# ocrickard/piper-swift

Hardware: AMD Instinct MI355X
Metric: audio-sec/wall-sec (RTF^-1) with ms/utterance, Piper VITS en_GB-medium geometry, scale-bench factor (higher is better)
Workload: dtype f32; 1 GPU; medium factor=8: 112 ids, 336 frames, 86016 samples (3.901 s audio) per utterance, 1 utterance per step per GPU; factor=8, phoneme_count=112, frames=336, samples=86016, parallelism=utterance-replicas x1 (one-shot RCCL weight broadcast)

## Files before the change

piper-swift_amd/csrc/rb_pair.hip:

```cpp
#include <algorithm>
#include <type_traits>

#include "conv_win.h"

namespace ph {
namespace {

typedef float f32x16 __attribute__((ext_vector_type(16)));

constexpr int kRA = 8;
constexpr int kStepPad = 16;
constexpr int kWN = 4, kNTW = 2, kT1 = kWN * kNTW;
constexpr int kColsA = 32 * kT1;
__host__ __device__ constexpr int halo_of(int pb) { return pb <= 16 ? 16 : 48; }
constexpr int kMaxReachB = 48;
constexpr int kStageU = 10;

struct RbPairMulti {
  RbPairArgs c[kWinMulti];
};

#ifdef PH_PAIR_TRACE
__device__ unsigned long long* ph_pair_trace_buf;
#define PH_STAMP(k) do { if (lane == 0 && round < 4 && ph_pair_trace_buf && blockIdx.x < 512) ph_pair_trace_buf[(((size_t)blockIdx.x * (MT * kWN) + wave) * 4 + round) * 8 + (k)] = __builtin_amdgcn_s_memtime(); } while (0)
#else
#define PH_STAMP(k) do { } while (0)
#endif

__device__ __forceinline__ float lrelu_max(float v, float alpha) { return fmaxf(v, v * alpha); }

__device__ __forceinline__ float bload(__amdgpu_buffer_rsrc_t r, int voff, int soff) {
  return __builtin_bit_cast(float, __builtin_amdgcn_raw_buffer_load_b32(r, voff, soff, 0));
}
__device__ __forceinline__ void bstore(__amdgpu_buffer_rsrc_t r, float v, int voff, int soff) {
  __builtin_amdgcn_raw_buffer_store_b32(__builtin_bit_cast(int, v), r, voff, soff, 0);
}

struct PairSched {
  int ntx[kWinMulti];
  int cnt[kWinMulti];
  int total, batch, order;
};

template <int MT>
__global__ __launch_bounds__(MT * kWN * 64, 2) void rb_pair_kernel(const RbPairMulti multi, const PairSched sch, const int Wx, const int W1,
                                                               const unsigned inv_w4) {
  extern __shared__ __attribute__((aligned(16))) float lds[];
  constexpr int BT = MT * kWN * 64;
  const int lane = threadIdx.x & 63;
  const int wave = __builtin_amdgcn_readfirstlane((int)(threadIdx.x >> 6));
  const int wm = wave % MT, wn = wave / MT;
  const int r = lane & 31, h = lane >> 5;
  constexpr int C = 32 * MT, C2 = C >> 1;
  float* xs = lds;
  float* x1s = lds + C * Wx + 4;
  float* biasS = x1s + C * W1;
  for (int i = threadIdx.x; i < kWinMulti * 2 * C; i += BT) {
    const int z = i / (2 * C), rem = i - z * 2 * C;
    const RbPairArgs& p = multi.c[(sch.order >> (4 * z)) & 15];
    biasS[i] = rem < C ? p.ba[rem] : p.bb[rem - C];
  }
  const int rowlane = wm * 32 + 4 * h;
  const unsigned lane16 = (unsigned)lane * 16u;
  const int G = (int)gridDim.x, bid = (int)blockIdx.x;

  struct Tile {
    const float *x, *wa4, *wb4;
    float* y;
    int bias_off;
    int Ka, dila, Kb, dilb, res_a, res_b_x, L, Lv, pa, pb, halo, c0, ga, shift, Sa, Spa, Sb, Spb, ntb;
    float alpha;
  };
  auto tile_index = [&](int round) {
    const int idx = round * G + ((round & 1) ? G - 1 - bid : bid);
    return idx < sch.total ? idx : -1;
  };
  auto setup = [&](int idx) {
    int z = 0, rem = idx;
    if (rem >= sch.cnt[0]) { rem -= sch.cnt[0]; z = 1; }
    if (z == 1 && rem >= sch.cnt[1]) { rem -= sch.cnt[1]; z = 2; }
    const RbPairArgs& p = multi.c[(sch.order >> (4 * z)) & 15];
    const int ntx = sch.ntx[z];
    const int n = __builtin_amdgcn_readfirstlane(rem / ntx);
    const int bx = rem - n * ntx;
    Tile t;
    t.x = p.x + (int64_t)n * C * p.L;
    t.y = p.y + (int64_t)n * C * p.L;
    t.wa4 = p.wa4; t.wb4 = p.wb4; t.bias_off = z * 2 * C;
    t.Ka = p.Ka; t.dila = p.dila; t.Kb = p.Kb; t.dilb = p.dilb; t.res_a = p.res_a; t.res_b_x = p.res_b_x; t.L = p.L; t.alpha = p.alpha;
    t.Lv = p.len_ptr ? min(p.len_ptr[n] * p.len_mul, p.L) : p.L;
    t.pa = (p.Ka - 1) * p.dila / 2; t.pb = (p.Kb - 1) * p.dilb / 2;
    t.halo = halo_of(t.pb);
    const int ncb = kColsA - 2 * t.halo;
    t.c0 = bx * ncb;
    const int g0 = t.c0 - t.halo - t.pa;
    t.ga = g0 & ~3;
    t.shift = g0 - t.ga;
    t.Sa = p.Ka * C2; t.Spa = (t.Sa + kStepPad - 1) / kStepPad * kStepPad;
    t.Sb = p.Kb * C2; t.Spb = (t.Sb + kStepPad - 1) / kStepPad * kStepPad;
    t.ntb = min(max((ncb >> 5) - wn * kNTW, 0), kNTW);
    return t;
  };

  float4 a[kRA];
  const char* wa = nullptr;
  auto load_a = [&](int slot, int ahead) { a[slot] = *(const float4*)(wa + ahead * 1024 + lane16); };
  auto ring_start = [&](const float* w4, int Sp) {
    wa = (const char*)w4 + (int64_t)wm * Sp * 256;
#pragma unroll
    for (int d = 0; d < kRA - 1; d++) load_a(d, d);
  };

  float4 pre[kStageU];
  const int W4 = Wx >> 2, total4 = C * W4;
  auto stage_issue = [&](const Tile& t, const int tx) {
#pragma unroll
    for (int u = 0; u < kStageU; u++) {
      const int ic = min(tx + u * BT, total4 - 1);
      const int row = (int)__umulhi((unsigned)ic, inv_w4);
      const int pos = t.ga + 4 * (ic - row * W4);
      pre[u] = *(const float4*)(t.x + (int64_t)row * t.L + ((pos >= 0 && pos < t.L) ? pos : 0));
    }
  };
  auto stage_commit = [&](const Tile& t, const int tx) {
#pragma unroll
    for (int u = 0; u < kStageU; u++) {
      const int i = tx + u * BT;
      const int ic = min(i, total4 - 1);
      const int row = (int)__umulhi((unsigned)ic, inv_w4);
      const int i4 = ic - row * W4;
      const int pos = t.ga + 4 * i4;
      const int nv = (pos >= 0 && pos < t.L) ? t.Lv - pos : 0;
      float4 v = pre[u];
      v.x = nv > 0 ? lrelu_max(v.x, t.alpha) : 0.0f; v.y = nv > 1 ? lrelu_max(v.y, t.alpha) : 0.0f;
      v.z = nv > 2 ? lrelu_max(v.z, t.alpha) : 0.0f; v.w = nv > 3 ? lrelu_max(v.w, t.alpha) : 0.0f;
      *(float4*)(xs + (i < total4 ? row * Wx + 4 * i4 : C * Wx)) = v;
    }
  };

  f32x16 acc[kNTW];
  auto run_conv = [&](auto nt_tag, const float* img, const int Wrow, const int S, const int Sp, const int dil, const int col0, const int bias_off) {
    constexpr int NT = decltype(nt_tag)::value;
#pragma unroll
    for (int g4 = 0; g4 < 4; g4++) {
      const float4 bv = *(const float4*)(biasS + bias_off + rowlane + 8 * g4);
#pragma unroll
      for (int j = 0; j < kNTW; j++) { acc[j][4 * g4] = bv.x; acc[j][4 * g4 + 1] = bv.y; acc[j][4 * g4 + 2] = bv.z; acc[j][4 * g4 + 3] = bv.w; }
    }
    const int lbase = h * Wrow + col0 + r;
    int sidx = 0, c_n = 0, left = S - 1;
    const int wrap_delta = dil - 2 * Wrow * (C2 - 1);
    float b[2][NT][4];
    auto read_b4 = [&](int slot) {
#pragma unroll
      for (int e = 0; e < 4; e++) {
#pragma unroll
        for (int j = 0; j < NT; j++) b[slot][j][e] = img[lbase + sidx + 32 * j];
        c_n++;
        const bool wrap = c_n == C2;
        c_n = wrap ? 0 : c_n;
        const int delta = wrap ? wrap_delta : 2 * Wrow;
        sidx += left > 0 ? delta : 0;
        left--;
      }
    };
    auto group = [&](int u) {
      load_a((u + kRA - 1) % kRA, kRA - 1 + u);
      read_b4((u + 1) & 1);
      __builtin_amdgcn_sched_barrier(0);
      const float av[4] = {a[u].x, a[u].y, a[u].z, a[u].w};
#pragma unroll
      for (int e = 0; e < 4; e++)
#pragma unroll
        for (int j = 0; j < NT; j++) acc[j] = __builtin_amdgcn_mfma_f32_32x32x2f32(av[e], b[u & 1][j][e], acc[j], 0, 0, 0);
    };
    read_b4(0);
    const int Gr = Sp >> 2, full = Gr / kRA;
    if (full > 0) {
#pragma unroll
      for (int u = 0; u < kRA; u++) group(u);
      wa += kRA * 1024;
    }
    for (int g = 1; g < full; g++) {
#pragma unroll
      for (int u = 0; u < kRA; u++) group(u);
      wa += kRA * 1024;
    }
    const int rem = Gr - full * kRA;
#pragma unroll
    for (int u = 0; u < kRA - 1; u++)
      if (u < rem) group(u);
  };

  Tile cur = setup(tile_index(0));
  ring_start(cur.wa4, cur.Spa);
  stage_issue(cur, (int)threadIdx.x);
  stage_commit(cur, (int)threadIdx.x);
  __syncthreads();

  for (int round = 0;; round++) {
    const int nidx = tile_index(round + 1);
    const bool has_next = nidx >= 0;
    const Tile nxt = has_next ? setup(nidx) : cur;
    int tx = (int)threadIdx.x, rl = rowlane, rr = r;
    asm volatile("" : "+v"(tx), "+v"(rl), "+v"(rr));
    float resx[kNTW][16];
    auto load_res = [&](int gres0) {
      const __amdgpu_buffer_rsrc_t rx = __builtin_amdgcn_make_buffer_rsrc((void*)cur.x, 0, C * cur.L * 4, 0x00020000);
#pragma unroll
      for (int j = 0; j < kNTW; j++) {
        const int g = gres0 + (wn * kNTW + j) * 32 + rr;
        const int voff = (g >= 0 && g < cur.L) ? (rl * cur.L + g) * 4 : -4;
#pragma unroll
        for (int q = 0; q < 16; q++) resx[j][q] = bload(rx, voff, ((q & 3) + 8 * (q >> 2)) * cur.L * 4);
      }
    };

    PH_STAMP(0);
    __builtin_amdgcn_s_waitcnt(0x0F70);
    PH_STAMP(1);
    if (has_next) stage_issue(nxt, tx);

    const bool live = cur.c0 < cur.Lv;
    if (live) run_conv(std::integral_constant<int, kNTW>{}, xs, Wx, cur.Sa, cur.Spa, cur.dila, cur.shift + wn * kNTW * 32, cur.bias_off);
    PH_STAMP(2);
    if (live) ring_start(cur.wb4, cur.Spb);
    if (live && cur.res_a) load_res(cur.c0 - cur.halo);
    __syncthreads();
    PH_STAMP(3);

    if (live) {
#pragma unroll
      for (int j = 0; j < kNTW; j++) {
        const int colw = (wn * kNTW + j) * 32 + rr;
        const int g = cur.c0 - cur.halo + colw;
        const bool in = g >= 0 && g < cur.Lv;
#pragma unroll
        for (int q = 0; q < 16; q++) {
          const int rq = (q & 3) + 8 * (q >> 2);
          const int o = (rl + rq) * W1 + colw;
          float v = acc[j][q];
          if (cur.res_a) v += resx[j][q];
          v = in ? v : 0.0f;
          x1s[o] = lrelu_max(v, cur.alpha);
          if (!cur.res_b_x) xs[o] = v;
        }
      }
    }
    __syncthreads();

    PH_STAMP(4);
    if (live && cur.ntb > 0) {
      const int col0b = cur.halo - cur.pb + wn * kNTW * 32;
      __builtin_amdgcn_s_waitcnt(0x0F70);
      if (cur.ntb == 2) run_conv(std::integral_constant<int, 2>{}, x1s, W1, cur.Sb, cur.Spb, cur.dilb, col0b, cur.bias_off + C);
      else run_conv(std::integral_constant<int, 1>{}, x1s, W1, cur.Sb, cur.Spb, cur.dilb, col0b, cur.bias_off + C);
    }
    PH_STAMP(5);
    if (has_next) ring_start(nxt.wa4, nxt.Spa);
    if (live && cur.res_b_x && cur.ntb > 0) load_res(cur.c0);
    if (live && cur.ntb > 0) {
      const __amdgpu_buffer_rsrc_t ry = __builtin_amdgcn_make_buffer_rsrc((void*)cur.y, 0, C * cur.L * 4, 0x00020000);
#pragma unroll
      for (int j = 0; j < kNTW; j++) {
        if (j >= cur.ntb) break;
        const int colo = (wn * kNTW + j) * 32 + rr;
        const int g = cur.c0 + colo;
        const int voff = g < cur.L ? (rl * cur.L + g) * 4 : -4;
#pragma unroll
        for (int q = 0; q < 16; q++) {
          const int rq = (q & 3) + 8 * (q >> 2);
          float v = acc[j][q];
          v += cur.res_b_x ? resx[j][q] : xs[(rl + rq) * W1 + cur.halo + colo];
          bstore(ry, v, voff, rq * cur.L * 4);
        }
      }
    }
    PH_STAMP(6);
    if (!has_next) break;
    __syncthreads();
    stage_commit(nxt, tx);
    __syncthreads();
    PH_STAMP(7);
    cur = nxt;
  }
}

struct PairGeom {
  int Wx, W1;
  size_t lds;
};

PairGeom pair_geom(int C, int pa_max, int pb_max) {
  auto pad = [](int w, bool odd32) {
    w = (w + 3) & ~3;
    if (odd32) while ((w & 63) != 32) w += 4;
    return w;
  };
  PairGeom g;
  for (int pass = 0; pass < 2; pass++) {
    g.Wx = pad(kColsA + 2 * pa_max + 3, pass == 0);
    g.W1 = pad(kColsA, pass == 0);
    (void)pb_max;
    g.lds = ((size_t)C * g.Wx + 4 + (size_t)C * g.W1 + (size_t)kWinMulti * 2 * C) * sizeof(float);
    if (g.lds <= 160 * 1024 && (C * g.Wx) / 4 <= kStageU * (C / 32) * kWN * 64) break;
  }
  return g;
}

template <int MT>
void launch_pair_inst(piper_hip_ctx* ctx, hipStream_t s, const RbPairMulti& m, const PairSched& sch, const PairGeom& g) {
  static bool raised[kMaxDevices] = {};
  if (g.lds > 64 * 1024 && lds_optin_needed(raised))
    (void)hipFuncSetAttribute((const void*)rb_pair_kernel<MT>, hipFuncAttributeMaxDynamicSharedMemorySize, 160 * 1024);
  const unsigned inv = (unsigned)(0x100000000ull / (unsigned)(g.Wx >> 2)) + 1u;
  const int per_cu = std::max(1, std::min(2, (int)((size_t)160 * 1024 / g.lds)));
  const int grid = std::min(sch.total, per_cu * ctx->num_cus);
  hipLaunchKernelGGL((rb_pair_kernel<MT>), dim3(grid), dim3(MT * kWN * 64), g.lds, s, m, sch, g.Wx, g.W1, inv);
}

}

#ifdef PH_PAIR_TRACE
void rb_pair_set_trace(unsigned long long* buf) { (void)hipMemcpyToSymbol(HIP_SYMBOL(ph_pair_trace_buf), &buf, sizeof buf); }
#endif

bool rb_pair_eligible(int C, int Ka, int dila, int Kb, int dilb, int L) {
  if (C != 32 && C != 64) return false;
  if (Ka < 1 || Kb < 1 || !(Ka & 1) || !(Kb & 1) || dila < 1 || dilb < 1) return false;
  if (L < 4 || (L & 3)) return false;
  const int pa = (Ka - 1) * dila / 2, pb = (Kb - 1) * dilb / 2;
  if (pb > kMaxReachB) return false;
  if ((int64_t)C * (kColsA + 2 * pa + 70) >= (1 << 20)) return false;
  const PairGeom g = pair_geom(C, pa, pb);
  return g.lds <= 160 * 1024 && (C * g.Wx) / 4 <= kStageU * (C / 32) * kWN * 64;
}

int launch_rb_pair_multi(piper_hip_ctx* ctx, hipStream_t s, const RbPairArgs* pairs, int count) {
  if (count < 1 || count > kWinMulti) PH_FAIL(PIPER_HIP_ERR_ARG, "rb_pair: %d pairs in one launch (1..%d)", count, kWinMulti);
  const RbPairArgs& a = pairs[0];
  if (a.N <= 0 || a.L <= 0) return PIPER_HIP_OK;
  int pa_max = 0, pb_max = 0;
  int idx[kWinMulti] = {0, 1, 2};
  for (int i = 0; i < count; i++) {
    const RbPairArgs& b = pairs[i];
    if (b.N != a.N || b.C != a.C || b.L != a.L) PH_FAIL(PIPER_HIP_ERR_SHAPE, "rb_pair: pairs of one launch must share N, C and L");
    if (!rb_pair_eligible(b.C, b.Ka, b.dila, b.Kb, b.dilb, b.L)) PH_FAIL(PIPER_HIP_ERR_UNSUPPORTED, "rb_pair: geometry not covered (C=%d K=%d,%d d=%d,%d L=%d)", b.C, b.Ka, b.Kb, b.dila, b.dilb, b.L);
    if (!(b.alpha > 0.0f && b.alpha < 1.0f)) PH_FAIL(PIPER_HIP_ERR_UNSUPPORTED, "rb_pair: LeakyReLU slope %g outside (0,1)", (double)b.alpha);
    if (!b.x || !b.y || !b.wa4 || !b.wb4 || !b.ba || !b.bb) PH_FAIL(PIPER_HIP_ERR_ARG, "rb_pair: null operand");
    pa_max = std::max(pa_max, (b.Ka - 1) * b.dila / 2);
    pb_max = std::max(pb_max, (b.Kb - 1) * b.dilb / 2);
  }
  const PairGeom g = pair_geom(a.C, pa_max, pb_max);
  if (g.lds > 160 * 1024 || (a.C * g.Wx) / 4 > kStageU * (a.C / 32) * kWN * 64)
    PH_FAIL(PIPER_HIP_ERR_UNSUPPORTED, "rb_pair: window of %zu bytes (row %d) exceeds LDS / the staging registers", g.lds, g.Wx);
  std::sort(idx, idx + count, [&](int l, int r2) { return pairs[l].Ka + pairs[l].Kb > pairs[r2].Ka + pairs[r2].Kb; });
  PairSched sch = {};
  sch.batch = a.N;
  for (int i = 0; i < count; i++) {
    const RbPairArgs& b = pairs[idx[i]];
    sch.order |= idx[i] << (4 * i);
    sch.ntx[i] = (int)ceil_div(a.L, kColsA - 2 * halo_of((b.Kb - 1) * b.dilb / 2));
    sch.cnt[i] = sch.ntx[i] * a.N;
    sch.total += sch.cnt[i];
  }
  for (int i = count; i < kWinMulti; i++) { sch.ntx[i] = 1; sch.cnt[i] = 0; }
  RbPairMulti m;
  for (int i = 0; i < kWinMulti; i++) m.c[i] = pairs[i < count ? i : 0];
  if (a.C == 32) launch_pair_inst<1>(ctx, s, m, sch, g);
  else launch_pair_inst<2>(ctx, s, m, sch, g);
  hipError_t e = hipGetLastError();
  if (e != hipSuccess) PH_FAIL(PIPER_HIP_ERR_LAUNCH, "rb_pair launch failed: %s", hipGetErrorString(e));
  return PIPER_HIP_OK;
}

}
namespace ph { namespace { PH_WARM(rb_pair, (rb_pair_kernel<1>)); } }
```

Measured before the change: 5570 audio-sec/wall-sec.

## Use exact conv-b halo per pair and interleave column tiles across waves

Tile halos for the fused residual-block pair are now sized exactly to conv b's reach instead of being rounded up to 16 or 48 columns, so each tile emits more output columns and fewer tiles are launched. A partial last 32-column group is kept only when it holds at least a minimum number of live columns. Conv-b column groups are interleaved across waves with a stride of 32*kWN so the variable output count spreads evenly, and stores are masked past the tile's output width. This trades recompute in the halo for reads past the x1 row edge, guarded by a static_assert that the over-read stays inside LDS. An env var switches back to the rounded halo.

```diff
diff --git a/piper-swift_amd/csrc/rb_pair.hip b/piper-swift_amd/csrc/rb_pair.hip
--- a/piper-swift_amd/csrc/rb_pair.hip
+++ b/piper-swift_amd/csrc/rb_pair.hip
@@ -12,8 +12,19 @@
 constexpr int kStepPad = 16;
 constexpr int kWN = 4, kNTW = 2, kT1 = kWN * kNTW;
 constexpr int kColsA = 32 * kT1;
-__host__ __device__ constexpr int halo_of(int pb) { return pb <= 16 ? 16 : 48; }
+#ifndef PH_PAIR_MIN_LIVE
+#define PH_PAIR_MIN_LIVE 16
+#endif
+constexpr int kMinLiveCols = PH_PAIR_MIN_LIVE;
+template <bool EXACT>
+__host__ __device__ constexpr int halo_of(int pb) { return EXACT ? pb : (pb <= 16 ? 16 : 48); }
+template <bool EXACT>
+__host__ __device__ constexpr int out_cols_of(int pb) {
+  const int n = kColsA - 2 * halo_of<EXACT>(pb);
+  return (n & 31) < kMinLiveCols ? n & ~31 : n;
+}
 constexpr int kMaxReachB = 48;
+static_assert(2 * kMaxReachB + 31 < kWinMulti * 2 * 32, "conv b's over-read past x1 column 255 must end inside the bias table");
 constexpr int kStageU = 10;
 
 struct RbPairMulti {
@@ -42,7 +53,7 @@
   int total, batch, order;
 };
 
-template <int MT>
+template <int MT, bool EXACT>
 __global__ __launch_bounds__(MT * kWN * 64, 2) void rb_pair_kernel(const RbPairMulti multi, const PairSched sch, const int Wx, const int W1,
                                                                const unsigned inv_w4) {
   extern __shared__ __attribute__((aligned(16))) float lds[];
@@ -61,6 +72,8 @@
     biasS[i] = rem < C ? p.ba[rem] : p.bb[rem - C];
   }
   const int rowlane = wm * 32 + 4 * h;
+  constexpr int kStrideB = EXACT ? 32 * kWN : 32;
+  const int tcol_a = wn * kNTW * 32, tcol_b = EXACT ? wn * 32 : tcol_a;
   const unsigned lane16 = (unsigned)lane * 16u;
   const int G = (int)gridDim.x, bid = (int)blockIdx.x;
 
@@ -68,7 +81,7 @@
     const float *x, *wa4, *wb4;
     float* y;
     int bias_off;
-    int Ka, dila, Kb, dilb, res_a, res_b_x, L, Lv, pa, pb, halo, c0, ga, shift, Sa, Spa, Sb, Spb, ntb;
+    int Ka, dila, Kb, dilb, res_a, res_b_x, L, Lv, pa, pb, halo, ncb, c0, ga, shift, Sa, Spa, Sb, Spb, ntb;
     float alpha;
   };
   auto tile_index = [&](int round) {
@@ -90,15 +103,16 @@
     t.Ka = p.Ka; t.dila = p.dila; t.Kb = p.Kb; t.dilb = p.dilb; t.res_a = p.res_a; t.res_b_x = p.res_b_x; t.L = p.L; t.alpha = p.alpha;
     t.Lv = p.len_ptr ? min(p.len_ptr[n] * p.len_mul, p.L) : p.L;
     t.pa = (p.Ka - 1) * p.dila / 2; t.pb = (p.Kb - 1) * p.dilb / 2;
-    t.halo = halo_of(t.pb);
-    const int ncb = kColsA - 2 * t.halo;
-    t.c0 = bx * ncb;
+    t.halo = halo_of<EXACT>(t.pb);
+    t.ncb = out_cols_of<EXACT>(t.pb);
+    t.c0 = bx * t.ncb;
     const int g0 = t.c0 - t.halo - t.pa;
     t.ga = g0 & ~3;
     t.shift = g0 - t.ga;
     t.Sa = p.Ka * C2; t.Spa = (t.Sa + kStepPad - 1) / kStepPad * kStepPad;
     t.Sb = p.Kb * C2; t.Spb = (t.Sb + kStepPad - 1) / kStepPad * kStepPad;
-    t.ntb = min(max((ncb >> 5) - wn * kNTW, 0), kNTW);
+    const int ntb_all = (t.ncb + 31) >> 5;
+    t.ntb = EXACT ? min(max((ntb_all - wn + kWN - 1) / kWN, 0), kNTW) : min(max(ntb_all - wn * kNTW, 0), kNTW);
     return t;
   };
 
@@ -139,8 +153,8 @@
   };
 
   f32x16 acc[kNTW];
-  auto run_conv = [&](auto nt_tag, const float* img, const int Wrow, const int S, const int Sp, const int dil, const int col0, const int bias_off) {
-    constexpr int NT = decltype(nt_tag)::value;
+  auto run_conv = [&](auto nt_tag, auto stride_tag, const float* img, const int Wrow, const int S, const int Sp, const int dil, const int col0, const int bias_off) {
+    constexpr int NT = decltype(nt_tag)::value, STRIDE = decltype(stride_tag)::value;
 #pragma unroll
     for (int g4 = 0; g4 < 4; g4++) {
       const float4 bv = *(const float4*)(biasS + bias_off + rowlane + 8 * g4);
@@ -155,7 +169,7 @@
 #pragma unroll
       for (int e = 0; e < 4; e++) {
 #pragma unroll
-        for (int j = 0; j < NT; j++) b[slot][j][e] = img[lbase + sidx + 32 * j];
+        for (int j = 0; j < NT; j++) b[slot][j][e] = img[lbase + sidx + STRIDE * j];
         c_n++;
         const bool wrap = c_n == C2;
         c_n = wrap ? 0 : c_n;
@@ -205,11 +219,11 @@
     int tx = (int)threadIdx.x, rl = rowlane, rr = r;
     asm volatile("" : "+v"(tx), "+v"(rl), "+v"(rr));
     float resx[kNTW][16];
-    auto load_res = [&](int gres0) {
+    auto load_res = [&](int gres0, int tcol, int stride) {
       const __amdgpu_buffer_rsrc_t rx = __builtin_amdgcn_make_buffer_rsrc((void*)cur.x, 0, C * cur.L * 4, 0x00020000);
 #pragma unroll
       for (int j = 0; j < kNTW; j++) {
-        const int g = gres0 + (wn * kNTW + j) * 32 + rr;
+        const int g = gres0 + tcol + stride * j + rr;
         const int voff = (g >= 0 && g < cur.L) ? (rl * cur.L + g) * 4 : -4;
 #pragma unroll
         for (int q = 0; q < 16; q++) resx[j][q] = bload(rx, voff, ((q & 3) + 8 * (q >> 2)) * cur.L * 4);
@@ -222,17 +236,17 @@
     if (has_next) stage_issue(nxt, tx);
 
     const bool live = cur.c0 < cur.Lv;
-    if (live) run_conv(std::integral_constant<int, kNTW>{}, xs, Wx, cur.Sa, cur.Spa, cur.dila, cur.shift + wn * kNTW * 32, cur.bias_off);
+    if (live) run_conv(std::integral_constant<int, kNTW>{}, std::integral_constant<int, 32>{}, xs, Wx, cur.Sa, cur.Spa, cur.dila, cur.shift + tcol_a, cur.bias_off);
     PH_STAMP(2);
     if (live) ring_start(cur.wb4, cur.Spb);
-    if (live && cur.res_a) load_res(cur.c0 - cur.halo);
+    if (live && cur.res_a) load_res(cur.c0 - cur.halo, tcol_a, 32);
     __syncthreads();
     PH_STAMP(3);
 
     if (live) {
 #pragma unroll
       for (int j = 0; j < kNTW; j++) {
-        const int colw = (wn * kNTW + j) * 32 + rr;
+        const int colw = tcol_a + j * 32 + rr;
         const int g = cur.c0 - cur.halo + colw;
         const bool in = g >= 0 && g < cur.Lv;
 #pragma unroll
@@ -251,22 +265,22 @@
 
     PH_STAMP(4);
     if (live && cur.ntb > 0) {
-      const int col0b = cur.halo - cur.pb + wn * kNTW * 32;
+      const int col0b = cur.halo - cur.pb + tcol_b;
       __builtin_amdgcn_s_waitcnt(0x0F70);
-      if (cur.ntb == 2) run_conv(std::integral_constant<int, 2>{}, x1s, W1, cur.Sb, cur.Spb, cur.dilb, col0b, cur.bias_off + C);
-      else run_conv(std::integral_constant<int, 1>{}, x1s, W1, cur.Sb, cur.Spb, cur.dilb, col0b, cur.bias_off + C);
+      if (cur.ntb == 2) run_conv(std::integral_constant<int, 2>{}, std::integral_constant<int, kStrideB>{}, x1s, W1, cur.Sb, cur.Spb, cur.dilb, col0b, cur.bias_off + C);
+      else run_conv(std::integral_constant<int, 1>{}, std::integral_constant<int, kStrideB>{}, x1s, W1, cur.Sb, cur.Spb, cur.dilb, col0b, cur.bias_off + C);
     }
     PH_STAMP(5);
     if (has_next) ring_start(nxt.wa4, nxt.Spa);
-    if (live && cur.res_b_x && cur.ntb > 0) load_res(cur.c0);
+    if (live && cur.res_b_x && cur.ntb > 0) load_res(cur.c0, tcol_b, kStrideB);
     if (live && cur.ntb > 0) {
       const __amdgpu_buffer_rsrc_t ry = __builtin_amdgcn_make_buffer_rsrc((void*)cur.y, 0, C * cur.L * 4, 0x00020000);
 #pragma unroll
       for (int j = 0; j < kNTW; j++) {
         if (j >= cur.ntb) break;
-        const int colo = (wn * kNTW + j) * 32 + rr;
+        const int colo = tcol_b + j * kStrideB + rr;
         const int g = cur.c0 + colo;
-        const int voff = g < cur.L ? (rl * cur.L + g) * 4 : -4;
+        const int voff = (colo < cur.ncb && g < cur.L) ? (rl * cur.L + g) * 4 : -4;
 #pragma unroll
         for (int q = 0; q < 16; q++) {
           const int rq = (q & 3) + 8 * (q >> 2);
@@ -308,15 +322,21 @@
   return g;
 }
 
-template <int MT>
+template <int MT, bool EXACT>
 void launch_pair_inst(piper_hip_ctx* ctx, hipStream_t s, const RbPairMulti& m, const PairSched& sch, const PairGeom& g) {
   static bool raised[kMaxDevices] = {};
   if (g.lds > 64 * 1024 && lds_optin_needed(raised))
-    (void)hipFuncSetAttribute((const void*)rb_pair_kernel<MT>, hipFuncAttributeMaxDynamicSharedMemorySize, 160 * 1024);
+    (void)hipFuncSetAttribute((const void*)rb_pair_kernel<MT, EXACT>, hipFuncAttributeMaxDynamicSharedMemorySize, 160 * 1024);
   const unsigned inv = (unsigned)(0x100000000ull / (unsigned)(g.Wx >> 2)) + 1u;
   const int per_cu = std::max(1, std::min(2, (int)((size_t)160 * 1024 / g.lds)));
   const int grid = std::min(sch.total, per_cu * ctx->num_cus);
-  hipLaunchKernelGGL((rb_pair_kernel<MT>), dim3(grid), dim3(MT * kWN * 64), g.lds, s, m, sch, g.Wx, g.W1, inv);
+  hipLaunchKernelGGL((rb_pair_kernel<MT, EXACT>), dim3(grid), dim3(MT * kWN * 64), g.lds, s, m, sch, g.Wx, g.W1, inv);
+}
+
+bool pair_exact_tiles(int C) {
+  static const bool rounded = getenv("PIPER_HIP_PAIR_HALO_ROUNDED") != nullptr;
+  (void)C;
+  return !rounded;
 }
 
 }
@@ -355,24 +375,26 @@
   if (g.lds > 160 * 1024 || (a.C * g.Wx) / 4 > kStageU * (a.C / 32) * kWN * 64)
     PH_FAIL(PIPER_HIP_ERR_UNSUPPORTED, "rb_pair: window of %zu bytes (row %d) exceeds LDS / the staging registers", g.lds, g.Wx);
   std::sort(idx, idx + count, [&](int l, int r2) { return pairs[l].Ka + pairs[l].Kb > pairs[r2].Ka + pairs[r2].Kb; });
+  const bool exact = pair_exact_tiles(a.C);
   PairSched sch = {};
   sch.batch = a.N;
   for (int i = 0; i < count; i++) {
     const RbPairArgs& b = pairs[idx[i]];
     sch.order |= idx[i] << (4 * i);
-    sch.ntx[i] = (int)ceil_div(a.L, kColsA - 2 * halo_of((b.Kb - 1) * b.dilb / 2));
+    const int pb = (b.Kb - 1) * b.dilb / 2;
+    sch.ntx[i] = (int)ceil_div(a.L, exact ? out_cols_of<true>(pb) : out_cols_of<false>(pb));
     sch.cnt[i] = sch.ntx[i] * a.N;
     sch.total += sch.cnt[i];
   }
   for (int i = count; i < kWinMulti; i++) { sch.ntx[i] = 1; sch.cnt[i] = 0; }
   RbPairMulti m;
   for (int i = 0; i < kWinMulti; i++) m.c[i] = pairs[i < count ? i : 0];
-  if (a.C == 32) launch_pair_inst<1>(ctx, s, m, sch, g);
-  else launch_pair_inst<2>(ctx, s, m, sch, g);
+  if (a.C == 32) exact ? launch_pair_inst<1, true>(ctx, s, m, sch, g) : launch_pair_inst<1, false>(ctx, s, m, sch, g);
+  else exact ? launch_pair_inst<2, true>(ctx, s, m, sch, g) : launch_pair_inst<2, false>(ctx, s, m, sch, g);
   hipError_t e = hipGetLastError();
   if (e != hipSuccess) PH_FAIL(PIPER_HIP_ERR_LAUNCH, "rb_pair launch failed: %s", hipGetErrorString(e));
   return PIPER_HIP_OK;
 }
 
 }
-namespace ph { namespace { PH_WARM(rb_pair, (rb_pair_kernel<1>)); } }
+namespace ph { namespace { PH_WARM(rb_pair, (rb_pair_kernel<1, true>)); } }
```

New measurement: 5773 audio-sec/wall-sec, median of 6. 1.04x the previous value.
